# baycom/tfrec

Hardware: AMD Instinct MI355X
Metric: IQ MSamples/s through demod+decode (batched streams) (higher is better)
Workload: dtype int32+f32+f64

## Files before the change

### tfrec_amd/csrc/chains2.hip

```cpp
#include <stdlib.h>

#include <algorithm>

#include "decoder_dev.h"
#include <type_traits>
#include "whb_chain_asm.h"

namespace tfrec {

constexpr int kSpecLbi = -(1 << 30);

__device__ __forceinline__ int whb_hook_perturb(const WinTables &T)
{
#ifdef TFREC_AMD_EXPERIMENTS
	return T.whb_test_perturb;
#else
	return 0;
#endif
}
__device__ __forceinline__ int whb_hook_force_fail(const WinTables &T)
{
#ifdef TFREC_AMD_EXPERIMENTS
	return T.whb_force_fail;
#else
	return 0;
#endif
}

__device__ __forceinline__ int tfa1_decay(int m) { return m - (int)(((uint32_t)m + 19u) / 20u); }

constexpr int kStatTfa1Scalar = 7, kStatTfa2Scalar = 8, kStatTfa1Vector = 9, kStatTfa2Vector = 10;
struct GroupStats {
	int scalar, vector;
};
__device__ __forceinline__ void stat_flush(const WinTables &T, const GroupStats &g, int slot_scalar, int slot_vector)
{
#if !defined(TFREC_AMD_COOPSTAT) && !defined(TFREC_AMD_VECSTAT) && !defined(TFREC_AMD_PROFILE_WHB)
	if ((threadIdx.x & 63) == 0) {
		if (g.scalar)
			atomicAdd(&T.stats[slot_scalar], (unsigned long long)g.scalar);
#ifdef TFREC_AMD_EXPERIMENTS
		if (g.vector)
			atomicAdd(&T.stats[slot_vector], (unsigned long long)g.vector);
#endif
	}
#endif
}

__device__ __forceinline__ int rebase_lbi(int lbi, int from_block, int to_block)
{
	return lbi ? lbi - kIndexSpan * (to_block - from_block) : 0;
}

struct BitWriter {
	uint32_t *base;
	uint32_t acc;
	int n;
	uint32_t pend;
	int pend_idx;
	__device__ __forceinline__ void put(int bit)
	{
		acc |= (uint32_t)bit << (n & 31);
		n++;
		if ((n & 31) == 0) {
			if (pend_idx >= 0)
				base[pend_idx] = pend;
			pend = acc;
			pend_idx = (n >> 5) - 1;
			acc = 0;
		}
	}
	__device__ __forceinline__ void put_bits(uint32_t v, int cnt)
	{
		const int sh = n & 31;
		const unsigned long long a = (unsigned long long)acc | ((unsigned long long)v << sh);
		n += cnt;
		if (sh + cnt >= 32) {
			if (pend_idx >= 0)
				base[pend_idx] = pend;
			pend = (uint32_t)a;
			pend_idx = (n >> 5) - 1;
			acc = (uint32_t)(a >> 32);
		} else {
			acc = (uint32_t)a;
		}
	}
	__device__ __forceinline__ void chunk_end()
	{
		const int idx = pend_idx >= 0 ? pend_idx : (n >> 5);
		base[idx] = pend_idx >= 0 ? pend : acc;
		pend_idx = -1;
	}
	__device__ __forceinline__ void finish()
	{
		chunk_end();
		if (n & 31)
			base[n >> 5] = acc;
	}
};

#include "windows.h"

#include "biquad.h"

#include "slicers.h"

#include "coop_slicer.h"

#include "whb_commit.h"

#include "whb_demod.h"

#include "whb_check.h"

#include "decode.h"

hipError_t launch_fmdev(hipStream_t st, const uint32_t *dec, size_t dec_stride, const unsigned long long *mask,
			size_t mask_stride, const uint32_t *prevdec, int16_t *fmdev, size_t fmdev_stride, EventBuf *eb,
			int n_streams, int n_blocks, int wmax, double flag_eps);

hipError_t launch_pipeline(const PipeCtl &P, const uint32_t *dec, size_t dec_stride, const unsigned long long *mask,
			   size_t mask_stride, const int16_t *fmdev, size_t fmdev_stride, int n_streams, int n_blocks,
			   long long sample_base, const ChainLaunch &L, const WinTables &T, int16_t *ld16, int32_t *dev32,
			   tfrec_amd_event *events, EventBuf *eb, uint32_t flags)
{
	auto mark = [&](int k, hipStream_t s_) {
		if (P.tev)
			(void)hipEventRecord(P.tev[k], s_);
	};
	hipError_t e = hipSuccess;
#define TRY(x)                          \
	do {                            \
		if ((e = (x)) != hipSuccess) \
			return e;       \
	} while (0)
	if (L.n_active == 0) {
		for (int k = 0; k < 3; k++)
			TRY(hipEventRecord(P.done[k], k == 0 ? P.cs : (k == 1 ? P.aux : P.t1)));
		return hipSuccess;
	}
	constexpr int lanes = 64;
	constexpr int head_chunks = 64;
	dim3 block(64);
	dim3 grid((n_streams + lanes - 1) / lanes, L.n_active);
	const int win_blocks = std::min(16384, (int)(((size_t)n_streams * n_blocks * 2 + lanes - 1) / lanes));
	const int seg_blocks = std::min(16384, (int)(((size_t)L.n_active * n_streams * ((size_t)n_blocks * (kBlockDec / 32) / kSegSlots + 4) +
						       lanes - 1) / lanes));
	const int repair_blocks = std::min(seg_blocks, std::max(256, seg_blocks / 8));
	const int spec_blocks = std::min(seg_blocks, std::max(256, seg_blocks / 5));
	const int long_window = (size_t)n_streams * L.n_active >= 1024 ? kLongWindow : kLongWindow / 2;
	const int coop_blocks = std::min(32768, std::max(1, (int)std::min<size_t>((size_t)L.n_active * n_streams *
								((size_t)n_blocks * kBlockDec / (size_t)long_window + 1), 1u << 30)));
	const int dec_blocks = std::min(16384, std::max(1, win_blocks));
	const bool has_whb = has_kind(L, 2), has_tfa2 = has_kind(L, 1), has_tfa1 = has_kind(L, 0);
	if (P.ws != P.fs)
		TRY(hipStreamWaitEvent(P.ws, P.ev_front, 0));
	TRY(hipMemsetAsync(T.queue, 0, (kNQueues + 1) * sizeof(WorkQueue), P.ws));
	mark(kMarkWindows, P.ws);
	hipLaunchKernelGGL(windows_kernel, dim3(n_streams), block, 0, P.ws, mask, mask_stride, n_streams, n_blocks, L, T,
			   long_window);
	mark(kMarkWindowsEnd, P.ws);
	TRY(hipEventRecord(P.ev_win, P.ws));
	int whb_spec = -1;
	if (has_whb) {
		TRY(hipStreamWaitEvent(P.kw, P.ev_win, 0));
		mark(kMarkWhbSpec, P.kw);
		hipLaunchKernelGGL((spec_biquad_kernel<true, 0>), dim3(spec_blocks), block, K3Tile<true>::kSize, P.kw, dec, dec_stride, fmdev, fmdev_stride,
				   n_streams, n_blocks, L, T, ld16, dev32, lanes);
		mark(kMarkWhbRepair, P.kw);
		hipLaunchKernelGGL((spec_biquad_kernel<true, 1>), dim3(repair_blocks), block, K3Tile<true>::kSize, P.kw, dec, dec_stride, fmdev, fmdev_stride,
				   n_streams, n_blocks, L, T, ld16, dev32, lanes);
		hipLaunchKernelGGL((spec_biquad_kernel<true, 2>), dim3(repair_blocks), block, K3Tile<true>::kSize, P.kw, dec, dec_stride, fmdev, fmdev_stride,
				   n_streams, n_blocks, L, T, ld16, dev32, lanes);
		mark(kMarkWhbFix, P.kw);
		hipLaunchKernelGGL(fix_biquad_kernel, dim3(n_streams, L.n_active), block, 0, P.kw, dec, dec_stride, fmdev, fmdev_stride,
				   n_streams, n_blocks, L, T, ld16, dev32, 2);
		mark(kMarkWhbBiquadEnd, P.kw);
		TRY(hipEventRecord(P.ev_kw, P.kw));
		TRY(hipStreamWaitEvent(P.aux, P.ev_kw, 0));
		mark(kMarkWhbDemod, P.aux);
		for (int a = 0; a < L.n_active; a++)
			if (L.params[a].kind == 2) {
				const dim3 wgrid(n_streams), wblock(64);
				const int wlds = 64 * 64;
				if (flags & TFREC_AMD_F_BITS) {
					hipLaunchKernelGGL((whb_demod_kernel<true, false>), wgrid, wblock, wlds, P.aux, dec, dec_stride, dev32, n_streams,
							   n_blocks, sample_base, L, a, T, events, eb, flags);
				} else {
					hipLaunchKernelGGL((whb_demod_kernel<false, false>), wgrid, wblock, wlds, P.aux, dec, dec_stride, dev32, n_streams,
							   n_blocks, sample_base, L, a, T, events, eb, flags);
					whb_spec = a;
				}
				mark(kMarkWhbDemodEnd, P.aux);
				mark(kMarkWhbDecodeEnd, P.aux);
				mark(kMarkWhbCommitEnd, P.aux);
			}
	}
	if (whb_spec >= 0) {
		if (P.vx != P.aux) {
			TRY(hipEventRecord(P.ev_aux, P.aux));
			TRY(hipStreamWaitEvent(P.vx, P.ev_aux, 0));
		}
		mark(kMarkWhbCheck, P.vx);
		hipLaunchKernelGGL(whb_chain_kernel, dim3((n_streams + kChkStreams - 1) / kChkStreams), dim3(64 * (1 + kChkProducers)), kChkLdsBytes,
				   P.vx, n_streams, L, whb_spec, T);
		hipLaunchKernelGGL(whb_check_kernel, dim3(n_streams), block, 0, P.vx, n_streams, L, whb_spec, T, P.whb_carry);
		ChainLaunch Lr = L;
		WinTables Tr = T;
		Tr.whbpub = L.states[whb_spec];
		Lr.states[whb_spec] = T.whbscr;
		hipLaunchKernelGGL((whb_demod_kernel<true, true>), dim3((n_streams + 63) / 64), block, 64 * 64, P.vx, dec, dec_stride, dev32, n_streams,
				   n_blocks, sample_base, Lr, whb_spec, Tr, events, eb, flags);
		mark(kMarkWhbCheckEnd, P.vx);
		TRY(hipEventRecord(P.done[1], P.vx));
	} else {
		TRY(hipEventRecord(P.done[1], P.aux));
	}
	static_assert(kMarkTfa2End == kMarkTfa2Coop + 3 && kMarkTfa1End == kMarkTfa1Coop + 3, "a slicer chain's marks are consecutive");
	auto slicer_chain = [&](int kind, hipStream_t s_, int m0) {
		if (kind == 0)
			hipLaunchKernelGGL(mark_kernel, dim3(std::max(1, win_blocks / 16)), dim3(256), 0, s_, dec, dec_stride, n_streams,
					   n_blocks, L, T);
		const size_t slds = (kind == 0 ? 8 : 4) * 64 * sizeof(uint4);
		hipLaunchKernelGGL(slicer_kernel, dim3(std::max(64, win_blocks)), block, slds, s_, dec, dec_stride, ld16, n_streams, n_blocks, L, T,
				   lanes, head_chunks, kind, 0);
		mark(m0, s_);
		hipLaunchKernelGGL(coop_slicer_kernel, dim3(coop_blocks), block, 0, s_, dec, dec_stride, ld16, n_streams, n_blocks, L,
				   T, kind);
		mark(m0 + 1, s_);
		hipLaunchKernelGGL(decode_kernel, dim3(dec_blocks), block, 0, s_, n_streams, L, T, kind);
		mark(m0 + 2, s_);
		hipLaunchKernelGGL(commit_kernel, grid, block, 0, s_, dec, dec_stride, ld16, n_streams, n_blocks, sample_base, L, T,
				   events, eb, flags, lanes, kind);
		if (kind == 1)
			hipLaunchKernelGGL(commit_wave_kernel, dim3(256), block, 0, s_, dec, dec_stride, ld16, n_streams, n_blocks,
					   sample_base, L, T, events, eb, flags);
		mark(m0 + 3, s_);
	};
	if (has_tfa2) {
		TRY(hipStreamWaitEvent(P.k2, P.ev_win, 0));
		if (P.fq && P.fmdev_wmax > 0) {
			TRY(hipStreamWaitEvent(P.fq, P.ev_front, 0));
			mark(kMarkFmdev, P.fq);
			TRY(launch_fmdev(P.fq, dec, dec_stride, mask, mask_stride, P.prevdec, P.fmdev_out, fmdev_stride, eb, n_streams,
					 n_blocks, P.fmdev_wmax, P.fm_flag_eps));
			mark(kMarkFmdevEnd, P.fq);
			TRY(hipEventRecord(P.ev_fm, P.fq));
			TRY(hipStreamWaitEvent(P.k2, P.ev_fm, 0));
		} else if (P.fmdev_wmax > 0) {
			mark(kMarkFmdev, P.k2);
			TRY(launch_fmdev(P.k2, dec, dec_stride, mask, mask_stride, P.prevdec, P.fmdev_out, fmdev_stride, eb, n_streams,
					 n_blocks, P.fmdev_wmax, P.fm_flag_eps));
			mark(kMarkFmdevEnd, P.k2);
		}
		hipStream_t sp = (P.ks && P.fq && P.fmdev_wmax > 0) ? P.ks : P.k2;
		if (sp != P.k2) {
			TRY(hipStreamWaitEvent(sp, P.ev_win, 0));
			TRY(hipStreamWaitEvent(sp, P.ev_fm, 0));
		}
		mark(kMarkTfa2Spec, sp);
		hipLaunchKernelGGL((spec_biquad_kernel<false, 0>), dim3(spec_blocks), block, K3Tile<false>::kSize, sp, dec, dec_stride, fmdev, fmdev_stride,
				   n_streams, n_blocks, L, T, ld16, dev32, lanes);
		mark(kMarkTfa2Repair, sp);
		if (sp != P.k2) {
			TRY(hipEventRecord(P.ev_spec, sp));
			TRY(hipStreamWaitEvent(P.k2, P.ev_spec, 0));
		}
		if (has_tfa1) {
			TRY(hipEventRecord(P.ev_fork, sp));
			TRY(hipStreamWaitEvent(P.t1, P.ev_fork, 0));
		}
		hipLaunchKernelGGL((spec_biquad_kernel<false, 1>), dim3(repair_blocks), block, K3Tile<false>::kSize, P.k2, dec, dec_stride, fmdev, fmdev_stride,
				   n_streams, n_blocks, L, T, ld16, dev32, lanes);
		hipLaunchKernelGGL((spec_biquad_kernel<false, 2>), dim3(repair_blocks), block, K3Tile<false>::kSize, P.k2, dec, dec_stride, fmdev, fmdev_stride,
				   n_streams, n_blocks, L, T, ld16, dev32, lanes);
		mark(kMarkTfa2Fix, P.k2);
		hipLaunchKernelGGL(fix_biquad_kernel, dim3(n_streams, L.n_active), block, 0, P.k2, dec, dec_stride, fmdev, fmdev_stride,
				   n_streams, n_blocks, L, T, ld16, dev32, 1);
		mark(kMarkTfa2BiquadEnd, P.k2);
		TRY(hipEventRecord(P.ev_k2, P.k2));
		TRY(hipStreamWaitEvent(P.cs, P.ev_k2, 0));
		mark(kMarkTfa2Slicer, P.cs);
		slicer_chain(1, P.cs, kMarkTfa2Coop);
	}
	TRY(hipEventRecord(P.done[0], P.cs));
	if (has_tfa1) {
		if (!has_tfa2)
			TRY(hipStreamWaitEvent(P.t1, P.ev_win, 0));
		mark(kMarkTfa1Slicer, P.t1);
		slicer_chain(0, P.t1, kMarkTfa1Coop);
	}
	TRY(hipEventRecord(P.done[2], P.t1));
#undef TRY
	return hipGetLastError();
}

hipError_t whb_chain_lds_optin()
{
	return hipFuncSetAttribute(reinterpret_cast<const void *>(&whb_chain_kernel), hipFuncAttributeMaxDynamicSharedMemorySize,
				   (int)kChkLdsBytes);
}

}
```

### tfrec_amd/csrc/whb_demod.h

```cpp
#pragma once

constexpr int kWhbSpb = 64, kWhbSpbShift = 6;
constexpr uint32_t kWhbSyncRev = 0xd2b42bd4u;

__device__ __forceinline__ int wave_shr1(int v)
{
	return __builtin_amdgcn_update_dpp(0, v, 0x138, 0xf, 0xf, false);
}
__device__ __forceinline__ void rows_replicate(int v, int (&out)[4])
{
	const auto r = __builtin_amdgcn_permlane16_swap(v, v, false, false);
	const auto e = __builtin_amdgcn_permlane32_swap(r[0], r[0], false, false);
	const auto o = __builtin_amdgcn_permlane32_swap(r[1], r[1], false, false);
	out[0] = e[0];
	out[1] = o[0];
	out[2] = e[1];
	out[3] = o[1];
}
__device__ __forceinline__ void rows_replicate(double v, double (&out)[4])
{
	int lo[4], hi[4];
	rows_replicate(__double2loint(v), lo);
	rows_replicate(__double2hiint(v), hi);
#pragma unroll
	for (int j = 0; j < 4; j++)
		out[j] = __hiloint2double(hi[j], lo[j]);
}
__device__ __forceinline__ double readlane_f64(double v, int lane)
{
	return __hiloint2double(__builtin_amdgcn_readlane(__double2hiint(v), lane), __builtin_amdgcn_readlane(__double2loint(v), lane));
}

template <int D>
__device__ __forceinline__ double row_shr_f64(double v)
{
	const int lo = __builtin_amdgcn_update_dpp(0, __double2loint(v), 0x110 + D, 0xf, 0xf, true);
	const int hi = __builtin_amdgcn_update_dpp(0, __double2hiint(v), 0x110 + D, 0xf, 0xf, true);
	return __hiloint2double(hi, lo);
}

struct WhbScan {
	double m2[4], m4[4], m8[4];
	double cy1, cy2;
	double ce[3][2];
	double a1;
};
__device__ __forceinline__ void whb_scan_init(WhbScan &w, double a1, double a2, int ln)
{
	w.a1 = a1;
	w.cy1 = w.cy2 = 0.0;
#pragma unroll
	for (int q = 0; q < 3; q++)
		w.ce[q][0] = w.ce[q][1] = 0.0;
	double gm2 = 0.0, gm1 = 0.0, g = 1.0;
	for (int n = 0; n <= 64; n++) {
		if (n == 2 || n == 4 || n == 8) {
			double *m = n == 2 ? w.m2 : (n == 4 ? w.m4 : w.m8);
			m[0] = g;
			m[1] = a2 * gm1;
			m[2] = gm1;
			m[3] = a2 * gm2;
		}
		if (n == ln + 1) {
			w.cy1 = g;
			w.cy2 = a2 * gm1;
		}
#pragma unroll
		for (int q = 0; q < 3; q++)
			if (n >= 1 && n == ln - 16 * q - 15) {
				w.ce[q][0] = g;
				w.ce[q][1] = a2 * gm1;
			}
		const double gn = a1 * g + a2 * gm1;
		gm2 = gm1;
		gm1 = g;
		g = gn;
	}
}
__device__ __forceinline__ double whb_scan_step(const WhbScan &w, double x, double y1, double y2)
{
	const double xs = row_shr_f64<1>(x);
	double u = __builtin_fma(w.a1, xs, x), v = xs;
	{
		const double us = row_shr_f64<2>(u), vs = row_shr_f64<2>(v);
		const double un = __builtin_fma(w.m2[0], us, __builtin_fma(w.m2[1], vs, u));
		v = __builtin_fma(w.m2[2], us, __builtin_fma(w.m2[3], vs, v));
		u = un;
	}
	{
		const double us = row_shr_f64<4>(u), vs = row_shr_f64<4>(v);
		const double un = __builtin_fma(w.m4[0], us, __builtin_fma(w.m4[1], vs, u));
		v = __builtin_fma(w.m4[2], us, __builtin_fma(w.m4[3], vs, v));
		u = un;
	}
	{
		const double us = row_shr_f64<8>(u), vs = row_shr_f64<8>(v);
		const double un = __builtin_fma(w.m8[0], us, __builtin_fma(w.m8[1], vs, u));
		v = __builtin_fma(w.m8[2], us, __builtin_fma(w.m8[3], vs, v));
		u = un;
	}
	double y = __builtin_fma(w.cy1, y1, __builtin_fma(w.cy2, y2, u));
#pragma unroll
	for (int q = 0; q < 3; q++) {
		const double eu = readlane_f64(u, 16 * q + 15), ev = readlane_f64(v, 16 * q + 15);
		y = __builtin_fma(w.ce[q][0], eu, __builtin_fma(w.ce[q][1], ev, y));
	}
	return y;
}

template <bool EXACT, bool REDO>
__global__ __launch_bounds__(64) void whb_demod_kernel(const uint32_t *__restrict__ dec, size_t dec_stride,
						       const int32_t *__restrict__ dev32, int n_streams, int n_blocks,
						       long long sample_base, ChainLaunch L, int a, WinTables T,
						       tfrec_amd_event *__restrict__ events, EventBuf *__restrict__ eb, uint32_t flags)
{
	constexpr bool redo = REDO;
	static_assert(EXACT || !REDO, "only the exact kernel redoes a submit");
	extern __shared__ __attribute__((aligned(16))) uint8_t rdata_lds[];
	__builtin_amdgcn_s_setprio(1);
	if (EXACT && !REDO)
		asm volatile("" ::: "v255", "a7");
	constexpr int kStep = 64;
	const int ln = threadIdx.x;
	auto stream_body = [&](const int s) {
	uint8_t *const rdata_wave = rdata_lds;
	const int c = a * n_streams + s;
	const int M = n_blocks * kBlockDec;
	const int count = T.count[c];
	constexpr int kStateChunks = (int)(sizeof(ChainState) / 16);
	static_assert(kStateChunks <= 64, "a wave copies a ChainState in one go");
	if (!EXACT) {
		const uint32_t gen = __atomic_load_n(&T.whbgen[s], __ATOMIC_RELAXED);
		__threadfence();
		if (ln < kStateChunks)
			reinterpret_cast<uint4 *>(&T.whbsnap[s])[ln] = reinterpret_cast<const uint4 *>(&L.states[a][s])[ln];
		if (ln == 0)
			T.whbseen[s] = gen;
	} else if (redo) {
		if (!T.whbfail[s])
			return;
		for (int j = ln; j < count; j += 64) {
			const int idx = T.result[(size_t)c * T.cap + j].first_cand_g;
			if (T.result[(size_t)c * T.cap + j].closed && idx >= 0 && (uint32_t)idx < eb->capacity) {
				events[idx].status = (uint8_t)kStatusDead;
				atomicAdd(&eb->dead, 1u);
			}
		}
		const bool stale = T.whbseen[s] != T.whbgen[s];
		const ChainState *from = stale ? &T.whbX[s] : &T.whbsnap[s];
		if (ln < kStateChunks)
			reinterpret_cast<uint4 *>(&L.states[a][s])[ln] = reinterpret_cast<const uint4 *>(from)[ln];
		__threadfence();
		__syncthreads();
		if (!stale && ln == 0) {
			const WhbExact x = T.whbx0[s];
			ChainState &st0 = L.states[a][s];
			st0.iir_avg.yn = x.y1;
			st0.iir_avg.yn1 = x.y2;
			st0.iir_avg.dn1 = 0.5 * (double)x.fd1;
			st0.iir_avg.dn2 = 0.5 * (double)x.fd2;
			st0.avg_of += x.carry;
		}
		__threadfence();
		__syncthreads();
	}
#ifdef TFREC_AMD_PROFILE_WHB
	long long pf_rec = 0, pf_steps = 0, pf_usteps = 0, pf_t0 = __builtin_readcyclecounter();
	long long pf_top = 0, pf_walk = 0, pf_tail = 0, pf_mark = 0;
	const long long pf_w0 = wall_clock64();
#endif
	if (count > 0) {
		const uint32_t *drow = dec + (size_t)s * dec_stride;
		const int32_t *dvrow = dev32 + (size_t)s * T.slots * 32;
		const ChainParams &p = L.params[a];
		ChainState &st = L.states[a][s];
		const double a1 = p.iir_avg.a1, a2 = p.iir_avg.a2;
		const double bh = 0.5 * p.iir_avg.b0;
		constexpr int tmin = 3 * kWhbSpb / 4 + 1;
		static_assert(kWhbSpb == 64 && (1 << kWhbSpbShift) == kWhbSpb && tmin > kStep / 2 && (kStep - 1 + kWhbSpb / 2) >> kWhbSpbShift == 1,
			      "the candidate walk knows two candidates per step, the second one bit long");
		auto sgpr = [](int v) -> int { return __builtin_amdgcn_readfirstlane(v); };
		auto sgpr64 = [](long long v) -> long long {
			const uint32_t lo = (uint32_t)__builtin_amdgcn_readfirstlane((int)(uint32_t)(unsigned long long)v);
			const uint32_t hi = (uint32_t)__builtin_amdgcn_readfirstlane((int)(uint32_t)((unsigned long long)v >> 32));
			return (long long)(((unsigned long long)hi << 32) | lo);
		};
		double y1 = st.iir_avg.yn, y2 = st.iir_avg.yn1;
		int fd1 = sgpr((int)(2.0 * st.iir_avg.dn1)), fd2 = sgpr((int)(2.0 * st.iir_avg.dn2));
		int avg_of = sgpr(st.avg_of), last_dev = sgpr(st.last_dev);
		long long step0 = sgpr64((long long)st.step);
		uint32_t since = (uint32_t)sgpr((int)(uint32_t)(st.step - st.last_peak));
		double rssi_d = st.rssi_d;
		int synced = sgpr(st.synced);
		uint32_t srr = (uint32_t)sgpr((int)__brev(st.sr));
		const uint32_t kmask = (uint32_t)sgpr((st.nrzs ^ st.w_last_bit) & 1 ? -1 : 0);
		uint32_t bhist = (uint32_t)sgpr((int)st.lfsr) ^ kmask;
		int sc = sgpr(st.sr_cnt), bc = sgpr(st.byte_cnt);
		const bool cont = T.cont[c] != 0;
		WhbScan scan;
		if (!EXACT)
			whb_scan_init(scan, a1, a2, ln);
		const int perturb = EXACT ? 0 : whb_hook_perturb(T);
		const int amb_tol = perturb > 1 ? perturb : (perturb < -1 ? -perturb : 1);
		const int amb_lo = amb_tol - 1;
		const uint32_t amb_w = 2u * (uint32_t)amb_tol;
		WhbStepRec *const recrow = T.whbrec + (size_t)s * T.whbrec_stride;
		int vstep = 0;
		int32_t *const dense = T.whbdense + (size_t)s * T.whbdense_stride;
		int dcount = 0;

		auto feed = [&](uint32_t e, int len) -> bool {
			const uint32_t emask = len >= 32 ? ~0u : (1u << len) - 1u;
			const uint32_t brun = __brev(e & emask) >> (32 - len);
			const unsigned long long hb = ((unsigned long long)bhist << len) | brun;
			const uint32_t orun = ((uint32_t)(hb ^ (hb >> 12) ^ (hb >> 17)) ^ kmask) & emask;
			const unsigned long long sv = ((unsigned long long)srr << len) | orun;
			const bool hit = ln < len && (uint32_t)(sv >> (len - 1 - (ln < len ? ln : 0))) == kWhbSyncRev;
			bhist = (uint32_t)hb;
			srr = (uint32_t)sv;
			return __ballot(hit) != 0ull;
		};

		for (int j = 0; j < count; j++) {
			const int og = sgpr(T.open[(size_t)c * T.cap + j]);
			const int close = sgpr(T.close[(size_t)c * T.cap + j]);
			const bool closed = close < M;
			const int n = (closed ? close : M - 1) - og + 1;
			const int nch = (n + kStep - 1) / kStep;
			const int slot0 = win_slot0(og, j);
			const int32_t *wq = dvrow + (size_t)slot0 * 32;
			uint16_t *ent = reinterpret_cast<uint16_t *>(T.bits + (size_t)c * T.bit_words + (og >> 6) + 3 * j);
			int ring0 = wq[ln], ring1 = wq[kStep + ln], ring2 = wq[2 * kStep + ln], ring3 = 0;
			wq += 3 * kStep;
			if (!(j == 0 && cont)) {
				rssi_d = 0;
				step0 = 0;
				since = 0;
			}
			const int vbase = vstep;
			int lock_pos = -1, avg_frozen = 0;
			bool amb = false;
			if (ln == 0) {
				WhbStart ws;
				ws.sr = __brev(srr);
				ws.lfsr = bhist ^ kmask;
				ws.sr_cnt = sc;
				ws.byte_cnt = bc;
				ws.synced = synced;
				ws.pad_[0] = ws.pad_[1] = ws.pad_[2] = 0;
				T.whbstart[(size_t)s * T.cap + j] = ws;
			}
			int nent = 0;
			auto put_ent = [&](uint32_t v16) {
				ent[nent] = (uint16_t)v16;
				nent++;
			};
			int rssi_from = synced ? 0 : -1;
			auto power_sum = [&](int from) -> unsigned long long {
				unsigned long long acc = 0ull;
#pragma unroll 4
				for (int m = from + ln; m < n; m += kStep) {
					const uint32_t w = drow[og + m];
					const int I = (int)(int16_t)(w & 0xffff), Q = (int)w >> 16;
					acc += (unsigned long long)(uint32_t)(I * I + Q * Q);
				}
#pragma unroll
				for (int o = 32; o >= 1; o >>= 1)
					acc += __shfl_xor(acc, o, 64);
				return acc;
			};
			auto step = [&](const int i, const int dev, int &fill) __attribute__((always_inline)) {
				const int nv = n - kStep * i < kStep ? n - kStep * i : kStep;
				const unsigned long long valid = nv < kStep ? (1ull << nv) - 1ull : ~0ull;
				fill = wq[ln];
				wq += kStep;
				const int sh1 = wave_shr1(dev);
				const int devm1 = ln == 0 ? last_dev : sh1;
				const unsigned long long rise_m = __builtin_amdgcn_ballot_w64(dev > devm1) & valid;
				const bool was_synced = synced != 0;
				unsigned long long mask;
				const double y1_in = y1;
				double ym = 0.0;
#ifdef TFREC_AMD_PROFILE_WHB
				pf_steps++;
				pf_mark = __builtin_readcyclecounter();
#endif
				const int fd1_in = fd1, fd2_in = fd2;
				const double y2_in = y2;
				auto scan_step = [&]() -> double {
					const int devm1f = ln == 0 ? fd1_in : sh1;
					const int sh2 = wave_shr1(devm1f);
					const int devm2f = ln == 0 ? fd2_in : sh2;
					const double t0 = bh * (double)dev, t1 = bh * (double)devm1f, t2 = bh * (double)devm2f;
					return whb_scan_step(scan, __builtin_fma(2.0, t1, t0) + t2, y1_in, y2_in);
				};
				if (!was_synced) {
#ifdef TFREC_AMD_PROFILE_WHB
					const long long pf_a = __builtin_readcyclecounter();
					pf_usteps++;
					pf_top += pf_a - pf_mark;
#endif
					if (EXACT) {
						const int devm1f = ln == 0 ? fd1 : sh1;
						const int sh2 = wave_shr1(devm1f);
						const int devm2f = ln == 0 ? fd2 : sh2;
						const double t0 = bh * (double)dev, t1 = bh * (double)devm1f, t2 = bh * (double)devm2f;
						const double ffp = __builtin_fma(2.0, t1, t0);
						double inp[4], inb[4];
						rows_replicate(ffp, inp);
						rows_replicate(t2, inb);
						double z0, z1, z2, z3, tt, tq, ya = 0.0, yb = 0.0, yc = y2, yd = y1;
						asm volatile(TFREC_WHB_CHAIN_ASM
							     : [Y0] "+v"(ya), [Y1] "+v"(yb), [Y2] "+v"(yc), [Y3] "+v"(yd), [Z0] "=&v"(z0), [Z1] "=&v"(z1),
							       [Z2] "=&v"(z2), [Z3] "=&v"(z3), [T] "=&v"(tt), [Q] "=&v"(tq)
							     : [a1] "s"(a1), [a2] "s"(a2), [ONE] "v"(1.0), [P0] "v"(inp[0]), [B0] "v"(inb[0]), [P1] "v"(inp[1]),
							       [B1] "v"(inb[1]), [P2] "v"(inp[2]), [B2] "v"(inb[2]), [P3] "v"(inp[3]), [B3] "v"(inb[3]));
						const int zq = ln & 3;
						ym = zq == 0 ? z0 : (zq == 1 ? z1 : (zq == 2 ? z2 : z3));
						if (nv == kStep) {
							y1 = yd;
							y2 = yc;
						} else {
							y1 = readlane_f64(ym, nv - 1);
							y2 = nv > 1 ? readlane_f64(ym, nv > 1 ? nv - 2 : 0) : y1_in;
						}
#ifdef TFREC_AMD_PROFILE_WHB
							pf_mark = __builtin_readcyclecounter();
							pf_rec += pf_mark - pf_a;
#endif
					} else {
						ym = scan_step();
						y1 = readlane_f64(ym, nv - 1);
						y2 = nv > 1 ? readlane_f64(ym, nv > 1 ? nv - 2 : 0) : y1_in;
#ifdef TFREC_AMD_PROFILE_WHB
						pf_mark = __builtin_readcyclecounter();
						pf_rec += pf_mark - pf_a;
#endif
					}
					const unsigned long long below = __builtin_amdgcn_ballot_w64(dev < (int)ym) & valid;
					if (!EXACT) {
						if (ln == 0) {
							WhbStepRec r;
							r.below = below;
							r.meta = (uint32_t)(slot0 + 2 * i) | ((uint32_t)(nv - 1) << kWhbRecNvShift);
							r.avgf = 0;
							recrow[vstep] = r;
						}
						vstep++;
					}
					mask = below & rise_m;
				} else {
					mask = __builtin_amdgcn_ballot_w64(dev < avg_of) & rise_m;
					if (!EXACT)
						amb = amb || (__builtin_amdgcn_ballot_w64((uint32_t)(avg_of + amb_lo - dev) < amb_w) & rise_m) != 0ull;
				}
				int locked_at = -1;
				auto pulse = [&](const int k, const int tdiff, auto ONE) {
					constexpr bool one = decltype(ONE)::value;
					const int bit0 = one ? 1 : (tdiff + kWhbSpb / 2) >> kWhbSpbShift;
					const int len = bit0 > 1 ? bit0 : 1;
					if (one || len < kWhbRunEsc) {
						put_ent((uint32_t)len);
					} else {
						put_ent((uint32_t)kWhbRunEsc);
						put_ent((uint32_t)len & 0xffffu);
						put_ent((uint32_t)len >> 16);
					}
					const int l0 = one ? 1 : (len < 32 ? len : 32);
					const unsigned long long hb = ((unsigned long long)bhist << l0) | ((1ull << (l0 - 1)) - 1ull);
					bool hit = false;
					if (synced == 0) {
						const uint32_t emask = (uint32_t)((1ull << l0) - 1ull);
						const uint32_t orun = ((uint32_t)hb ^ (uint32_t)(hb >> 12) ^ (uint32_t)(hb >> 17) ^ kmask) & emask;
						const unsigned long long sv = ((unsigned long long)srr << l0) | orun;
						if (one) {
							hit = (uint32_t)sv == kWhbSyncRev;
						} else {
							const unsigned long long hits = __builtin_amdgcn_ballot_w64((uint32_t)(sv >> ln) == kWhbSyncRev);
							hit = (hits & (unsigned long long)emask) != 0ull;
						}
						srr = (uint32_t)sv;
					}
					bhist = (uint32_t)hb;
					if (!one && len > 32)
						for (int rest = (len > 160 ? 160 : len) - 32; rest > 0; rest -= 32)
							hit = feed(~0u, rest < 32 ? rest : 32) || hit;
					if (synced == 0) {
						if (sc >= 0) {
							const int i0 = (8 - sc) & 7;
							bc += i0 < len ? (len - 1 - i0) / 8 + 1 : 0;
							sc = (sc + len) & 7;
						}
						if (hit) {
							synced = 1;
							locked_at = k;
							const double yk = readlane_f64(ym, k), ykm1 = readlane_f64(ym, k > 0 ? k - 1 : 0);
							const int dk = __builtin_amdgcn_readlane(dev, k);
							const int dkm1 = __builtin_amdgcn_readlane(dev, k > 0 ? k - 1 : 0);
							y2 = k > 0 ? ykm1 : y1_in;
							y1 = yk;
							fd2 = k > 0 ? dkm1 : fd1;
							fd1 = dk;
							avg_of = (int)yk + perturb;
							lock_pos = kStep * i + k;
							avg_frozen = avg_of;
							const unsigned long long after = k < kStep - 1 ? ~0ull << (k + 1) : 0ull;
							mask = __builtin_amdgcn_ballot_w64(dev < avg_of) & rise_m & after;
							if (!EXACT)
								amb = amb || (__builtin_amdgcn_ballot_w64((uint32_t)(avg_of + amb_lo - dev) < amb_w) & rise_m & after) != 0ull;
						}
					}
				};
				if (mask) {
					const int kmin = (int)since < -kStep ? kStep : tmin - (int)since;
					const unsigned long long m1 = kmin > 0 ? (kmin > kStep - 1 ? 0ull : mask & (~0ull << kmin)) : mask;
					if (m1) {
						const int k = __builtin_ctzll(m1);
						pulse(k, (int)(since + (uint32_t)k), std::false_type{});
						since = (uint32_t)-k;
						const int k2min = k + tmin;
						const unsigned long long m2 = k2min > kStep - 1 ? 0ull : mask & (~0ull << k2min);
						if (m2) {
							const int k2 = __builtin_ctzll(m2);
							pulse(k2, k2 - k, std::true_type{});
							since = (uint32_t)-k2;
						}
					}
				}
#ifdef TFREC_AMD_PROFILE_WHB
				{
					const long long t = __builtin_readcyclecounter();
					pf_walk += t - pf_mark;
					pf_mark = t;
				}
#endif
				const int dl1 = __builtin_amdgcn_readlane(dev, nv - 1);
				if (!EXACT && !was_synced) {
					const int nvf = locked_at >= 0 ? locked_at + 1 : nv;
					if (ln < nvf)
						dense[dcount + ln] = dev;
					dcount += nvf;
				}
				if (!was_synced && locked_at < 0) {
					fd2 = nv > 1 ? __builtin_amdgcn_readlane(dev, nv > 1 ? nv - 2 : 0) : fd1;
					fd1 = dl1;
					avg_of = (int)y1;
				}
				last_dev = dl1;
				since += (uint32_t)nv;
				if (locked_at >= 0)
					rssi_from = kStep * i + locked_at;
#ifdef TFREC_AMD_PROFILE_WHB
				pf_tail += __builtin_readcyclecounter() - pf_mark;
#endif
			};
			for (int i = 0; i < nch; i += 4) {
				step(i, ring0, ring3);
				if (i + 1 >= nch)
					break;
				step(i + 1, ring1, ring0);
				if (i + 2 >= nch)
					break;
				step(i + 2, ring2, ring1);
				if (i + 3 >= nch)
					break;
				step(i + 3, ring3, ring2);
			}
			WinResult res;
			res.nbits = nent;
			res.closed = 0;
			long long rssi_out = 0;
			if (closed) {
				if (synced) {
					const unsigned long long tot = power_sum(rssi_from);
					(void)feed(0u, 16);
					rssi_out = (long long)(rssi_d + (double)tot);
					res.closed = 1;
					srr = 0;
					synced = 0;
					sc = -1;
					bc = 0;
				}
				rssi_d = 0;
				step0 = 0;
				since = 0;
			} else {
				if (synced)
					rssi_d += (double)power_sum(rssi_from);
				step0 += n;
			}
			res.rssi_i = (int32_t)(uint32_t)((unsigned long long)rssi_out & 0xffffffffull);
			res.offset = (int32_t)(uint32_t)((unsigned long long)rssi_out >> 32);
			res.lbi_out = 0;
			res.first_cand_g = -1;
			res.bitcnt = vstep - vbase;
			res.dmax = lock_pos;
			res.dmin = avg_frozen;
			res.mark_lvl = vbase;
			res.last_bit = amb ? 1 : 0;
			res.resume = -1;
			if (ln == 0)
				T.result[(size_t)c * T.cap + j] = res;
			if (!EXACT) {
				const uint32_t wfl = (amb ? kWhbRecAmb : 0u) | (res.closed ? kWhbRecClosed : 0u);
				if (lock_pos >= 0) {
					if (ln == 0) {
						WhbStepRec *r = &recrow[vbase + (lock_pos >> 6)];
						r->meta = (uint32_t)(slot0 + 2 * (lock_pos >> 6)) | ((uint32_t)(lock_pos & 63) << kWhbRecNvShift) | kWhbRecLock | wfl;
						r->avgf = avg_frozen;
					}
				} else if (vstep == vbase) {
					if (ln == 0) {
						WhbStepRec r;
						r.below = 0ull;
						r.meta = kWhbRecPseudo | wfl;
						r.avgf = 0;
						recrow[vstep] = r;
					}
					vstep++;
				}
			}
		}
		if (!EXACT && ln == 0) {
			WhbStepRec r;
			r.below = 0ull;
			r.meta = kWhbRecEnd;
			r.avgf = 0;
			recrow[vstep] = r;
			T.whbdense_n[s] = dcount;
		}
		if (ln == 0) {
			const uint32_t lw = drow[M - 1];
			st.prev_i = (int)(int16_t)(lw & 0xffff);
			st.prev_q = (int)lw >> 16;
			st.timeout_cnt = T.timeout_next[c];
			st.last_dev = last_dev;
			st.avg_of = avg_of;
			st.step = (unsigned long long)step0;
			st.last_peak = (unsigned long long)(step0 - since);
			st.rssi_d = rssi_d;
			st.iir_avg.yn = y1;
			st.iir_avg.yn1 = y2;
			st.iir_avg.dn1 = 0.5 * (double)fd1;
			st.iir_avg.dn2 = 0.5 * (double)fd2;
		}
	} else if (ln == 0) {
		if (!EXACT) {
			WhbStepRec r;
			r.below = 0ull;
			r.meta = kWhbRecEnd;
			r.avgf = 0;
			T.whbrec[(size_t)s * T.whbrec_stride] = r;
			T.whbdense_n[s] = 0;
		}
		ChainState &st = L.states[a][s];
		const uint32_t lw = dec[(size_t)s * dec_stride + M - 1];
		st.prev_i = (int)(int16_t)(lw & 0xffff);
		st.prev_q = (int)lw >> 16;
		st.timeout_cnt = T.timeout_next[c];
	}
#ifdef TFREC_AMD_PROFILE_WHB
	if (ln == 0) {
#ifndef TFREC_AMD_PROFILE_WHB_SPAN
		atomicAdd(&T.stats[5], (unsigned long long)pf_rec);
#endif
#ifdef TFREC_AMD_PROFILE_WHB_SPAN
		if (sample_base == 5LL * n_blocks * kBlockDec) {
			atomicMax(&T.stats[1], ~(unsigned long long)pf_w0);
			atomicMax(&T.stats[2], (unsigned long long)pf_w0);
			atomicMax(&T.stats[3], (unsigned long long)wall_clock64());
			atomicAdd(&T.stats[0], (unsigned long long)pf_w0 & 0xffffffffffull);
			atomicMax(&T.stats[5], ((unsigned long long)(__builtin_readcyclecounter() - pf_t0) << 24) | (unsigned long long)pf_steps);
			{
				const long long cps = (__builtin_readcyclecounter() - pf_t0) / (pf_steps > 0 ? pf_steps : 1) / 100;
				const int b = cps < 25 ? 0 : (cps < 30 ? 1 : (cps < 35 ? 2 : (cps < 45 ? 3 : 4)));
				atomicAdd(&T.stats[6], 1ull << (12 * b));
			}
		}
#else
		atomicAdd(&T.stats[1], (unsigned long long)pf_top);
		atomicAdd(&T.stats[2], (unsigned long long)pf_walk);
		atomicAdd(&T.stats[3], (unsigned long long)pf_tail);
#endif
		atomicAdd(&T.stats[7], (unsigned long long)(__builtin_readcyclecounter() - pf_t0));
#ifndef TFREC_AMD_PROFILE_WHB_SPAN
		atomicAdd(&T.stats[6], (unsigned long long)(wall_clock64() - pf_w0));
#endif
		atomicAdd(&T.stats[4], (unsigned long long)((pf_steps << 32) | pf_usteps));
	}
#endif
	__threadfence();
	__syncthreads();
	for (int j = ln; j < count; j += 64)
		whb_decode_window(s, j, n_streams, L, a, T, rdata_wave + 64 * ln);
	__threadfence();
	__syncthreads();
	if (ln == 0)
		whb_commit_stream(s, n_streams, n_blocks, sample_base, L, a, T, events, eb, flags, rdata_wave);
	if (EXACT && redo) {
		__threadfence();
		__syncthreads();
		constexpr int kIirChunk0 = (int)(offsetof(ChainState, iir) / 16), kIirChunk1 = (int)(offsetof(ChainState, iir_avg) / 16);
		static_assert(offsetof(ChainState, iir) % 16 == 0 && offsetof(ChainState, iir_avg) % 16 == 0, "ChainState::iir must fill whole 16-byte chunks");
		if (ln < kStateChunks) {
			const uint4 v = reinterpret_cast<const uint4 *>(&L.states[a][s])[ln];
			reinterpret_cast<uint4 *>(&T.whbX[s])[ln] = v;
			if (ln < kIirChunk0 || ln >= kIirChunk1)
				reinterpret_cast<uint4 *>(&T.whbpub[s])[ln] = v;
		}
		__threadfence();
		__syncthreads();
		if (ln == 0) {
			const ChainState &st1 = L.states[a][s];
			WhbExact x;
			x.y1 = st1.iir_avg.yn;
			x.y2 = st1.iir_avg.yn1;
			x.fd1 = (int)(2.0 * st1.iir_avg.dn1);
			x.fd2 = (int)(2.0 * st1.iir_avg.dn2);
			x.carry = x.pad_ = 0;
			T.whbx[s] = x;
			T.whbfail[s] = 0;
			__threadfence();
			atomicAdd(&T.whbgen[s], 1u);
			atomicAdd(&T.stats[6], 1ull);
		}
	}
	};
	if (!REDO) {
		stream_body((int)blockIdx.x);
	} else {
		for (int base = 64 * (int)blockIdx.x; base < n_streams; base += 64 * (int)gridDim.x) {
			unsigned long long m = __ballot(base + ln < n_streams && T.whbfail[base + ln] != 0);
			while (m) {
				const int k = __builtin_ctzll(m);
				m &= m - 1;
				stream_body(base + k);
				__syncthreads();
			}
		}
	}
}
```

Before: 298,700.

## Stage WHB demod dense, step-record and entry writes in LDS rings, flush in bursts

The WHB demod kernel used to write dense deviation values, per-step records and pulse entries straight to global memory as scattered per-lane or lane-0 stores. These now go into LDS ring buffers and are flushed as wide, coalesced vector stores once a burst threshold is reached, with a tail flush at the end. The aim is to replace many small uncoalesced global stores with fewer full-wave transactions. In exchange it adds LDS traffic, branch checks on every step, and a larger dynamic LDS allocation. The ring bookkeeping is also delicate, for example a lock record that is patched after it may already have been flushed.

```diff
diff --git a/tfrec_amd/csrc/chains2.hip b/tfrec_amd/csrc/chains2.hip
--- a/tfrec_amd/csrc/chains2.hip
+++ b/tfrec_amd/csrc/chains2.hip
@@ -182,7 +182,7 @@
 		for (int a = 0; a < L.n_active; a++)
 			if (L.params[a].kind == 2) {
 				const dim3 wgrid(n_streams), wblock(64);
-				const int wlds = 64 * 64;
+				const int wlds = kWhbLdsBytes;
 				if (flags & TFREC_AMD_F_BITS) {
 					hipLaunchKernelGGL((whb_demod_kernel<true, false>), wgrid, wblock, wlds, P.aux, dec, dec_stride, dev32, n_streams,
 							   n_blocks, sample_base, L, a, T, events, eb, flags);
@@ -209,7 +209,7 @@
 		WinTables Tr = T;
 		Tr.whbpub = L.states[whb_spec];
 		Lr.states[whb_spec] = T.whbscr;
-		hipLaunchKernelGGL((whb_demod_kernel<true, true>), dim3((n_streams + 63) / 64), block, 64 * 64, P.vx, dec, dec_stride, dev32, n_streams,
+		hipLaunchKernelGGL((whb_demod_kernel<true, true>), dim3((n_streams + 63) / 64), block, kWhbLdsBytes, P.vx, dec, dec_stride, dev32, n_streams,
 				   n_blocks, sample_base, Lr, whb_spec, Tr, events, eb, flags);
 		mark(kMarkWhbCheckEnd, P.vx);
 		TRY(hipEventRecord(P.done[1], P.vx));
diff --git a/tfrec_amd/csrc/whb_demod.h b/tfrec_amd/csrc/whb_demod.h
--- a/tfrec_amd/csrc/whb_demod.h
+++ b/tfrec_amd/csrc/whb_demod.h
@@ -2,6 +2,22 @@
 
 constexpr int kWhbSpb = 64, kWhbSpbShift = 6;
 constexpr uint32_t kWhbSyncRev = 0xd2b42bd4u;
+
+constexpr int kWhbBurst = 256;
+constexpr int kWhbDenseRing = 2 * kWhbBurst;
+constexpr int kWhbRecRing = 8, kWhbRecBurst = 4;
+constexpr int kWhbEntRing = 128, kWhbEntBurst = 64;
+constexpr int kWhbStageBytes = kWhbDenseRing * 4 + kWhbRecRing * 16 + kWhbEntRing * 2;
+constexpr int kWhbLdsBytes = kWhbStageBytes > 64 * 64 ? kWhbStageBytes : 64 * 64;
+static_assert(kWhbBurst % 64 == 0 && (kWhbDenseRing & (kWhbDenseRing - 1)) == 0 && kWhbEntBurst % 2 == 0, "whole aligned bursts, rings indexed by mask");
+typedef uint32_t whb_u32x4 __attribute__((ext_vector_type(4)));
+typedef __attribute__((address_space(1))) whb_u32x4 whb_global_u32x4;
+typedef __attribute__((address_space(1))) uint32_t whb_global_u32;
+typedef __attribute__((address_space(1))) uint16_t whb_global_u16;
+__device__ __forceinline__ void whb_burst_mark()
+{
+	asm volatile("; whb_burst" ::: "memory");
+}
 
 __device__ __forceinline__ int wave_shr1(int v)
 {
@@ -208,6 +224,18 @@
 		int vstep = 0;
 		int32_t *const dense = T.whbdense + (size_t)s * T.whbdense_stride;
 		int dcount = 0;
+		int32_t *const stg_dense = reinterpret_cast<int32_t *>(rdata_lds);
+		WhbStepRec *const stg_rec = reinterpret_cast<WhbStepRec *>(rdata_lds + kWhbDenseRing * 4);
+		uint16_t *const stg_ent = reinterpret_cast<uint16_t *>(rdata_lds + kWhbDenseRing * 4 + kWhbRecRing * 16);
+		int dflushed = 0, vflushed = 0;
+		auto put_rec = [&](unsigned long long below, uint32_t meta) {
+			WhbStepRec r;
+			r.below = below;
+			r.meta = meta;
+			r.avgf = 0;
+			stg_rec[vstep & (kWhbRecRing - 1)] = r;
+			vstep++;
+		};
 
 		auto feed = [&](uint32_t e, int len) -> bool {
 			const uint32_t emask = len >= 32 ? ~0u : (1u << len) - 1u;
@@ -250,10 +278,39 @@
 				ws.pad_[0] = ws.pad_[1] = ws.pad_[2] = 0;
 				T.whbstart[(size_t)s * T.cap + j] = ws;
 			}
-			int nent = 0;
+			int nent = 0, eflushed = 0;
 			auto put_ent = [&](uint32_t v16) {
-				ent[nent] = (uint16_t)v16;
+				stg_ent[nent & (kWhbEntRing - 1)] = (uint16_t)v16;
 				nent++;
+			};
+			auto burst = [&]() __attribute__((always_inline)) {
+				if (!EXACT && dcount - dflushed >= kWhbBurst) {
+					whb_burst_mark();
+#pragma unroll
+					for (int q = 0; q < kWhbBurst; q += 256) {
+						const int k = dflushed + q + 4 * ln;
+						if (kWhbBurst % 256 == 0 || 4 * ln < kWhbBurst - q)
+							*(whb_global_u32x4 *)(uintptr_t)(dense + k) = *reinterpret_cast<const whb_u32x4 *>(stg_dense + (k & (kWhbDenseRing - 1)));
+					}
+					dflushed += kWhbBurst;
+					whb_burst_mark();
+				}
+				if (!EXACT && vstep - vflushed > kWhbRecBurst) {
+					whb_burst_mark();
+					if (ln < kWhbRecBurst)
+						*(whb_global_u32x4 *)(uintptr_t)(recrow + vflushed + ln) =
+							*reinterpret_cast<const whb_u32x4 *>(stg_rec + ((vflushed + ln) & (kWhbRecRing - 1)));
+					vflushed += kWhbRecBurst;
+					whb_burst_mark();
+				}
+				if (nent - eflushed >= kWhbEntBurst) {
+					whb_burst_mark();
+					const int k = (eflushed >> 1) + ln;
+					if (ln < kWhbEntBurst / 2)
+						*((whb_global_u32 *)(uintptr_t)ent + k) = reinterpret_cast<const uint32_t *>(stg_ent)[k & (kWhbEntRing / 2 - 1)];
+					eflushed += kWhbEntBurst;
+					whb_burst_mark();
+				}
 			};
 			int rssi_from = synced ? 0 : -1;
 			auto power_sum = [&](int from) -> unsigned long long {
@@ -277,6 +334,7 @@
 				const int sh1 = wave_shr1(dev);
 				const int devm1 = ln == 0 ? last_dev : sh1;
 				const unsigned long long rise_m = __builtin_amdgcn_ballot_w64(dev > devm1) & valid;
+				burst();
 				const bool was_synced = synced != 0;
 				unsigned long long mask;
 				const double y1_in = y1;
@@ -338,16 +396,8 @@
 #endif
 					}
 					const unsigned long long below = __builtin_amdgcn_ballot_w64(dev < (int)ym) & valid;
-					if (!EXACT) {
-						if (ln == 0) {
-							WhbStepRec r;
-							r.below = below;
-							r.meta = (uint32_t)(slot0 + 2 * i) | ((uint32_t)(nv - 1) << kWhbRecNvShift);
-							r.avgf = 0;
-							recrow[vstep] = r;
-						}
-						vstep++;
-					}
+					if (!EXACT)
+						put_rec(below, (uint32_t)(slot0 + 2 * i) | ((uint32_t)(nv - 1) << kWhbRecNvShift));
 					mask = below & rise_m;
 				} else {
 					mask = __builtin_amdgcn_ballot_w64(dev < avg_of) & rise_m;
@@ -437,8 +487,7 @@
 				const int dl1 = __builtin_amdgcn_readlane(dev, nv - 1);
 				if (!EXACT && !was_synced) {
 					const int nvf = locked_at >= 0 ? locked_at + 1 : nv;
-					if (ln < nvf)
-						dense[dcount + ln] = dev;
+					stg_dense[(dcount + ln) & (kWhbDenseRing - 1)] = dev;
 					dcount += nvf;
 				}
 				if (!was_synced && locked_at < 0) {
@@ -501,33 +550,32 @@
 			res.resume = -1;
 			if (ln == 0)
 				T.result[(size_t)c * T.cap + j] = res;
+			whb_burst_mark();
+			for (int k = eflushed + ln; k < nent; k += 64)
+				*((whb_global_u16 *)(uintptr_t)ent + k) = stg_ent[k & (kWhbEntRing - 1)];
+			whb_burst_mark();
 			if (!EXACT) {
 				const uint32_t wfl = (amb ? kWhbRecAmb : 0u) | (res.closed ? kWhbRecClosed : 0u);
 				if (lock_pos >= 0) {
-					if (ln == 0) {
-						WhbStepRec *r = &recrow[vbase + (lock_pos >> 6)];
-						r->meta = (uint32_t)(slot0 + 2 * (lock_pos >> 6)) | ((uint32_t)(lock_pos & 63) << kWhbRecNvShift) | kWhbRecLock | wfl;
-						r->avgf = avg_frozen;
-					}
+					WhbStepRec *r = &stg_rec[(vbase + (lock_pos >> 6)) & (kWhbRecRing - 1)];
+					r->meta = (uint32_t)(slot0 + 2 * (lock_pos >> 6)) | ((uint32_t)(lock_pos & 63) << kWhbRecNvShift) | kWhbRecLock | wfl;
+					r->avgf = avg_frozen;
 				} else if (vstep == vbase) {
-					if (ln == 0) {
-						WhbStepRec r;
-						r.below = 0ull;
-						r.meta = kWhbRecPseudo | wfl;
-						r.avgf = 0;
-						recrow[vstep] = r;
-					}
-					vstep++;
-				}
-			}
-		}
-		if (!EXACT && ln == 0) {
-			WhbStepRec r;
-			r.below = 0ull;
-			r.meta = kWhbRecEnd;
-			r.avgf = 0;
-			recrow[vstep] = r;
-			T.whbdense_n[s] = dcount;
+					put_rec(0ull, kWhbRecPseudo | wfl);
+				}
+			}
+		}
+		if (!EXACT) {
+			put_rec(0ull, kWhbRecEnd);
+			whb_burst_mark();
+			for (int k = dflushed + ln; k < dcount; k += 64)
+				*((whb_global_u32 *)(uintptr_t)dense + k) = (uint32_t)stg_dense[k & (kWhbDenseRing - 1)];
+			if (ln < vstep - vflushed)
+				*(whb_global_u32x4 *)(uintptr_t)(recrow + vflushed + ln) =
+					*reinterpret_cast<const whb_u32x4 *>(stg_rec + ((vflushed + ln) & (kWhbRecRing - 1)));
+			whb_burst_mark();
+			if (ln == 0)
+				T.whbdense_n[s] = dcount;
 		}
 		if (ln == 0) {
 			const uint32_t lw = drow[M - 1];
```

New measurement: 297,600. No clear change (-0.4%).
